# sunxiaojun2014/cilium

Hardware: AMD Instinct MI355X
Metric: Mpps classified (LPM ipcache + policy map) at 1/2/4/8 GPUs; % HBM roofline (higher is better)
Workload: dtype u32; 1 GPU; config2: 100k IPv4 ipcache LPM + 64k policy entries (4 ep x 16k), 64M-tuple batches per GPU, bit-exact verdicts; tuples_per_gpu=67108864

## Files before the change

### cilium_amd/_abi.py

```python
from __future__ import annotations

import ctypes as C
import os

HERE = os.path.dirname(os.path.abspath(__file__))
LIB_PATH = os.path.join(HERE, "libcgpu.so")

CGPU_ABI_VERSION = 2


class CgpuConfig(C.Structure):
    _fields_ = [
        ("abi_version", C.c_uint32),
        ("ipcache_max", C.c_uint32), ("policy_max_per_ep", C.c_uint32),
        ("policy_max_total", C.c_uint32), ("max_endpoints", C.c_uint32),
        ("cidr_dyn_max", C.c_uint32), ("cidr_fix_max", C.c_uint32),
        ("endpoints_max", C.c_uint32),
        ("host_id", C.c_uint32), ("world_id", C.c_uint32), ("cluster_id", C.c_uint32),
        ("health_id", C.c_uint32),
        ("ipv4_cluster_mask", C.c_uint32), ("ipv4_cluster_range", C.c_uint32),
        ("ipv6_router_ip", C.c_uint8 * 16),
        ("ct_proto_gate", C.c_uint8), ("ingress_secctx_world", C.c_uint8),
        ("prefilter_fix4", C.c_uint8), ("prefilter_dyn4", C.c_uint8),
        ("prefilter_fix6", C.c_uint8), ("prefilter_dyn6", C.c_uint8),
# ... 150 lines not shown
    "cgpu_cidr_update": (i32, [vp, i32, vp, u64]),
    "cgpu_cidr_delete": (i32, [vp, i32, vp]),
    "cgpu_cidr_lookup": (i32, [vp, i32, vp]),
    "cgpu_cidr_get_next_key": (i32, [vp, i32, vp, vp]),
    "cgpu_cidr_update_batch": (i32, [vp, i32, vp, sz, u64]),
    "cgpu_prefilter_insert": (i32, [vp, C.c_int64, vp, sz]),
    "cgpu_prefilter_delete": (i32, [vp, C.c_int64, vp, sz]),
    "cgpu_prefilter_revision": (i32, [vp, C.POINTER(C.c_int64)]),
    "cgpu_endpoint_update": (i32, [vp, vp, u64]),
    "cgpu_endpoint_delete": (i32, [vp, vp]),
    "cgpu_endpoint_lookup": (i32, [vp, vp]),
    "cgpu_endpoint_update_info": (i32, [vp, vp, vp, u64]),
    "cgpu_endpoint_lookup_info": (i32, [vp, vp, vp]),
    "cgpu_tunnel_update": (i32, [vp, vp, vp, u64]),
    "cgpu_tunnel_delete": (i32, [vp, vp]),
    "cgpu_tunnel_lookup": (i32, [vp, vp, vp]),
    "cgpu_tunnel_get_next_key": (i32, [vp, vp, vp]),
    "cgpu_tunnel_count": (sz, [vp]),
    "cgpu_forward_v4": (i32, [vp, C.POINTER(FwdParams), C.POINTER(FwdIn), sz, C.POINTER(FwdOut), vp]),
    "cgpu_forward_v6": (i32, [vp, C.POINTER(FwdParams), C.POINTER(FwdIn), sz, C.POINTER(FwdOut), vp]),
    "cgpu_forward_table_bytes": (i32, [vp, vp]),
    "cgpu_forward_frames": (i32, [vp, C.POINTER(FwdfParams), C.POINTER(FwdfIn), sz, C.POINTER(FwdOut), vp]),
    "cgpu_deliver_v4": (i32, [vp, C.POINTER(DlvIn), sz, C.POINTER(DlvOut), vp]),
    "cgpu_deliver_v6": (i32, [vp, C.POINTER(DlvIn), sz, C.POINTER(DlvOut), vp]),
    "cgpu_lb4_update": (i32, [vp, vp, vp, u64]),
    "cgpu_lb4_update_batch": (i32, [vp, vp, vp, sz, u64]),
    "cgpu_lb4_delete": (i32, [vp, vp]),
    "cgpu_lb4_lookup": (i32, [vp, vp, vp]),
    "cgpu_lb4_get_next_key": (i32, [vp, vp, vp]),
    "cgpu_lb4_count": (sz, [vp]),
    "cgpu_lb6_update": (i32, [vp, vp, vp, u64]),
    "cgpu_lb6_update_batch": (i32, [vp, vp, vp, sz, u64]),
    "cgpu_lb6_delete": (i32, [vp, vp]),
    "cgpu_lb6_lookup": (i32, [vp, vp, vp]),
    "cgpu_lb6_get_next_key": (i32, [vp, vp, vp]),
    "cgpu_lb6_count": (sz, [vp]),
    "cgpu_revnat4_update": (i32, [vp, u16, vp, u64]),
    "cgpu_revnat4_delete": (i32, [vp, u16]),
    "cgpu_revnat4_lookup": (i32, [vp, u16, vp]),
    "cgpu_revnat4_get_next_key": (i32, [vp, C.POINTER(u16), C.POINTER(u16)]),
    "cgpu_revnat4_count": (sz, [vp]),
    "cgpu_revnat6_update": (i32, [vp, u16, vp, u64]),
    "cgpu_revnat6_delete": (i32, [vp, u16]),
    "cgpu_revnat6_lookup": (i32, [vp, u16, vp]),
    "cgpu_revnat6_get_next_key": (i32, [vp, C.POINTER(u16), C.POINTER(u16)]),
    "cgpu_revnat6_count": (sz, [vp]),
    "cgpu_flow_hash6": (u32, [vp, vp, C.c_uint16, C.c_uint16, C.c_uint8]),
    "cgpu_flow_hash": (u32, [u32, u32, C.c_uint16, C.c_uint16, C.c_uint8]),
    "cgpu_commit": (i32, [vp, C.POINTER(u64)]),
    "cgpu_table_checksum": (i32, [vp, C.POINTER(u64)]),
    "cgpu_table_verify": (i32, [vp]),
    "cgpu_mirror_save": (i32, [vp, C.c_char_p]),
    "cgpu_mirror_restore": (i32, [vp, C.c_char_p]),
    "cgpu__test_corrupt": (i32, [vp, i32, sz, C.c_uint8]),
    "cgpu_counter_layout_checksum": (i32, [vp, C.POINTER(u64)]),
    "cgpu_classify_v4": (i32, [vp, C.POINTER(TuplesV4), sz, vp, vp, vp, vp]),
    "cgpu_classify_v4_host": (i32, [vp, C.POINTER(TuplesV4), sz, vp, vp, vp, vp]),
    "cgpu_classify_v6": (i32, [vp, C.POINTER(TuplesV6), sz, vp, vp, vp, vp]),
    "cgpu_classify_v4_tun": (i32, [vp, C.POINTER(TuplesV4), vp, vp, i32, sz, vp, vp, vp, vp, vp]),
    "cgpu_classify_v6_tun": (i32, [vp, C.POINTER(TuplesV6), vp, vp, i32, sz, vp, vp, vp, vp, vp]),
    "cgpu_classify_v6_lb": (i32, [vp, C.POINTER(TuplesV6), vp, vp, sz, vp, vp, vp, vp]),
    "cgpu_classify_v4_lb": (i32, [vp, C.POINTER(TuplesV4), vp, vp, sz, vp, vp, vp, vp]),
    "cgpu_classify_v4_cascade": (i32, [vp, C.POINTER(TuplesV4), vp, vp, sz, vp, vp, vp, vp]),
    "cgpu_classify_v4_lb_host": (i32, [vp, C.POINTER(TuplesV4), vp, vp, sz, vp, vp, vp, vp]),
    "cgpu_classify_v4_cascade_host": (i32, [vp, C.POINTER(TuplesV4), vp, vp, sz, vp, vp, vp, vp]),
    "cgpu_classify_v6_host": (i32, [vp, C.POINTER(TuplesV6), sz, vp, vp, vp, vp]),
    "cgpu_classify_v6_lb_host": (i32, [vp, C.POINTER(TuplesV6), vp, vp, sz, vp, vp, vp, vp]),
    "cgpu_lb4_select": (i32, [vp, i32, C.POINTER(Lb4Tuples), sz, C.POINTER(Lb4Out), vp]),
    "cgpu_prefilter_v4": (i32, [vp, vp, vp, vp, sz, vp, vp]),
    "cgpu_prefilter_v6": (i32, [vp, vp, vp, vp, sz, vp, vp]),
    "cgpu_prefilter_v4_host": (i32, [vp, vp, vp, vp, sz, vp, vp]),
    "cgpu_prefilter_v6_host": (i32, [vp, vp, vp, vp, sz, vp, vp]),
    "cgpu_lxc_update": (i32, [vp, u32, vp]),
    "cgpu_lxc_delete": (i32, [vp, u32]),
    "cgpu_lxc_lookup": (i32, [vp, u32, vp]),
    "cgpu_frames_parse": (i32, [vp, C.POINTER(Frames), sz, C.POINTER(FrameTuples), vp]),
    "cgpu_classify_frames": (i32, [vp, C.POINTER(Frames), sz, vp, vp, vp, vp]),
    "cgpu_classify_frames_host": (i32, [vp, C.POINTER(Frames), sz, vp, vp, vp, vp]),
    "cgpu_classify_frames_lb": (i32, [vp, C.POINTER(FlbIn), u32, sz, vp, vp, vp, C.POINTER(FlbOut), vp]),
    "cgpu_ct4_update": (i32, [vp, vp, vp, u64]),
    "cgpu_ct4_delete": (i32, [vp, vp]),
    "cgpu_ct4_lookup": (i32, [vp, vp, vp]),
    "cgpu_ct4_get_next_key": (i32, [vp, vp, vp]),
    "cgpu_ct4_count": (sz, [vp]),
    "cgpu_ct4_gc": (i32, [vp, u32, C.POINTER(u64)]),
    "cgpu_ct_stats": (i32, [vp, C.c_int, vp]),
    "cgpu_ct_lru_stats": (i32, [vp, C.c_int, vp]),
    "cgpu_ct4_flush": (i32, [vp]),
    "cgpu_classify_v4_ct": (i32, [vp, C.POINTER(TuplesV4Ct), sz, u32, vp, vp, vp, vp, vp]),
    "cgpu_classify_v4_ct_tun": (i32, [vp, C.POINTER(TuplesV4Ct), sz, u32, vp, vp, vp, vp, vp, vp]),
    "cgpu_classify_v6_ct_tun": (i32, [vp, C.POINTER(TuplesV6Ct), sz, u32, vp, vp, vp, vp, vp, vp]),
    "cgpu_classify_v4_ctlb": (i32, [vp, C.POINTER(TuplesV4Ct), vp, sz, u32, C.POINTER(CtlbOut), vp]),
    "cgpu_ct6_update": (i32, [vp, vp, vp, u64]),
    "cgpu_ct6_delete": (i32, [vp, vp]),
    "cgpu_ct6_lookup": (i32, [vp, vp, vp]),
    "cgpu_ct6_get_next_key": (i32, [vp, vp, vp]),
    "cgpu_ct6_count": (sz, [vp]),
    "cgpu_ct6_gc": (i32, [vp, u32, C.POINTER(u64)]),
    "cgpu_ct6_flush": (i32, [vp]),
    "cgpu_classify_v6_ctlb": (i32, [vp, C.POINTER(TuplesV6Ct), vp, sz, u32, C.POINTER(CtlbOut), vp]),
    "cgpu_classify_v6_ct": (i32, [vp, C.POINTER(TuplesV6Ct), sz, u32, vp, vp, vp, vp, vp]),
    "cgpu_classify_v4_ct_rnat": (i32, [vp, C.POINTER(TuplesV4Ct), sz, u32, vp, vp, vp, vp,
                                       C.POINTER(Rnat4Out), vp]),
    "cgpu_classify_v4_ctlb_rnat": (i32, [vp, C.POINTER(TuplesV4Ct), vp, sz, u32, C.POINTER(CtlbOut),
                                         C.POINTER(Rnat4Out), vp]),
    "cgpu_classify_v6_ct_rnat": (i32, [vp, C.POINTER(TuplesV6Ct), sz, u32, vp, vp, vp, vp,
                                       C.POINTER(Rnat6Out), vp]),
    "cgpu_classify_v6_ctlb_rnat": (i32, [vp, C.POINTER(TuplesV6Ct), vp, sz, u32, C.POINTER(CtlbOut),
                                         C.POINTER(Rnat6Out), vp]),
    "cgpu_rnat_frames_v4": (i32, [vp, C.POINTER(Rnf4In), u32, sz, vp, vp]),
    "cgpu_rnat_frames_v6": (i32, [vp, C.POINTER(Rnf6In), u32, sz, vp, vp]),
    "cgpu_frames_parse_ct": (i32, [vp, C.POINTER(Frames), sz, C.POINTER(FrameCtCols), vp]),
    "cgpu_classify_frames_ct": (i32, [vp, C.POINTER(Frames), sz, u32, C.POINTER(FctOut), vp]),
    "cgpu_l3_compile":(i32, [vp, vp, vp, vp, u32, vp]),
    "cgpu_mapstate_sync": (i32, [vp, vp, vp, vp, vp, vp]),
    "cgpu_counter_delta_bytes": (sz, [vp]),
    "cgpu_counter_bind": (i32, [vp, vp, sz]),
    "cgpu_counter_fold": (i32, [vp, vp]),
    "cgpu_metrics_read": (i32, [vp, vp]),
    "cgpu_counters_reset": (i32, [vp]),
    "cgpu_stream_release": (i32, [vp, vp]),
    "cgpu_host_stage_release": (i32, [vp]),
    "cgpu_table_bytes": (i32, [vp, vp]),
    "cgpu_host_stage_bytes": (sz, [vp]),
    "cgpu_counters_rebalance": (i32, [vp, C.POINTER(u64)]),
    "cgpu_comm_id_create": (i32, [vp]),
    "cgpu_comm_init": (i32, [vp, vp, i32, i32]),
    "cgpu_counters_allreduce": (i32, [vp, vp]),
}

_lib = None


class CgpuLibraryMissing(RuntimeError):
    pass


def lib():
    global _lib
    if _lib is None:
        if not os.path.exists(LIB_PATH):
            raise CgpuLibraryMissing(
                f"{LIB_PATH} is missing: build it with `python -m cilium_amd.build` "
                "(there is no CPU fallback for the classification path)")
        L = C.CDLL(LIB_PATH)
        for name, (res, args) in PROTOS.items():
            f = getattr(L, name)
            f.restype = res
            f.argtypes = args
        _lib = L
    return _lib


class CgpuError(OSError):
    pass


def check(rc: int, what: str) -> int:
    if rc < 0:
        msg = lib().cgpu_last_error().decode(errors="replace")
        raise CgpuError(-rc, f"{what}: {os.strerror(-rc)} ({msg})")
    return rc
```

### cilium_amd/csrc/host.cpp

```cpp
#include <hip/hip_runtime.h>
#include <rccl/rccl.h>

#include <algorithm>
#include <array>
#include <cerrno>
#include <cstdarg>
#include <cstdio>
#include <cstdlib>
#include <cstring>
#include <deque>
#include <functional>
#include <map>
#include <memory>
#include <mutex>
#include <thread>
#include <set>
#include <string>
#include <type_traits>
#include <unordered_map>
#include <vector>

#include "../../include/cgpu.h"
#include "launch.h"
#include "tables.h"
// ... 94 lines not shown
};
struct PolEntry {
	uint16_t proxy_port;
	uint32_t slot;
	uint64_t first_epoch;
};
struct SlotInit {
	uint32_t slot;
	uint64_t packets, bytes;
};

struct Dir248 {
	std::vector<uint32_t> tbl24, tbl8, vals;
	bool share = false;
	std::unordered_map<uint32_t, uint32_t> shared;
	void init() { tbl24.assign(DIR_TBL24_ENTRIES, 0u); tbl8.clear(); vals.clear(); shared.clear(); }
	uint32_t encode(uint32_t label)
	{
		if (label < (1u << DIR_TAG_SHIFT))
			return DIR_TAG_DIRECT | label;
		if (share) {
			auto it = shared.find(label);
			if (it != shared.end())
				return DIR_TAG_INDIRECT | it->second;
			shared.emplace(label, (uint32_t)vals.size());
		}
		vals.push_back(label);
		return DIR_TAG_INDIRECT | (uint32_t)(vals.size() - 1);
	}
	void apply(uint32_t addr, uint32_t len, uint32_t enc)
	{
		if (len <= 24) {
			uint32_t cnt = 1u << (24 - len);
			uint32_t base = len == 0 ? 0 : ((addr >> 8) & ~(cnt - 1));
			std::fill(tbl24.begin() + base, tbl24.begin() + base + cnt, enc);
			return;
		}
		uint32_t idx = addr >> 8, e = tbl24[idx];
		if ((e & DIR_TAG_MASK) != DIR_TAG_GROUP) {
			uint32_t g = (uint32_t)(tbl8.size() / 256);
			tbl8.resize(tbl8.size() + 256, e);
			tbl24[idx] = DIR_TAG_GROUP | g;
		}
		uint32_t g = tbl24[idx] & DIR_PAYLOAD_MASK;
		uint32_t cnt = 1u << (32 - len);
		uint32_t lo = (addr & 255u) & ~(cnt - 1);
		std::fill(tbl8.begin() + g * 256 + lo, tbl8.begin() + g * 256 + lo + cnt, enc);
	}
};

struct Lpm16cBuild {
	std::vector<uint32_t> d16, nodes, x16, dict;
	std::unordered_map<uint32_t, uint32_t> code;
	size_t nodes_at_build = 0;
	typedef std::vector<std::pair<uint32_t, uint32_t>> Runs;
	static void push(Runs &r, uint32_t start, uint32_t v)
	{
		if (r.empty() || r.back().second != v)
			r.push_back({start, v});
	}
	uint32_t emit_node(const Runs &r)
	{
		const uint32_t k = (uint32_t)r.size() - 1;
		const uint32_t kind = k <= 2 ? 0u : (k <= 4 ? 1u : 2u);
		const uint32_t nb = kind == 0 ? 1u : (kind == 1 ? 2u : 5u);
		const uint32_t words = kind == 0 ? 4u : (kind == 1 ? 8u : 16u);
		const uint32_t off = (uint32_t)(nodes.size() / 4);
		nodes.resize(nodes.size() + words, 0u);
		uint32_t *w = &nodes[(size_t)off * 4];
		for (uint32_t i = 0; i < 2 * nb; i++) {
			uint32_t b = i < k ? r[i + 1].first : 0xFFFFu;
			w[i / 2] |= (i & 1) ? (b << 16) : b;
		}
		for (uint32_t i = 0; i <= 2 * nb && nb + i < words; i++)
			w[nb + i] = r[std::min<uint32_t>(i, k)].second;
		return DIR_TAG_GROUP | (kind << LPMC_KIND_SHIFT) | off;
	}
	uint32_t emit_array(const uint32_t *ent)
	{
		const uint32_t off = (uint32_t)(nodes.size() / 4);
		nodes.insert(nodes.end(), ent, ent + 256);
		return DIR_TAG_GROUP | (3u << LPMC_KIND_SHIFT) | off;
	}
	uint32_t byte_level(const uint32_t *leaf)
	{
		Runs r;
		for (uint32_t j = 0; j < 256; j++)
			push(r, j, leaf[j]);
		if (r.size() == 1)
			return r[0].second;
		if (r.size() - 1 <= LPMC_MAX_RUN_BOUNDS)
			return emit_node(r);
		return emit_array(leaf);
	}
	static Runs runs16(uint32_t p, const std::vector<uint32_t> &tbl24, const std::vector<uint32_t> &tbl8)
	{
		Runs r;
		const uint32_t *t = &tbl24[(size_t)p * 256];
		for (uint32_t j = 0; j < 256 && r.size() <= LPMC_MAX_RUN_BOUNDS + 1; j++) {
			if ((t[j] & DIR_TAG_MASK) != DIR_TAG_GROUP) {
				push(r, j << 8, t[j]);
				continue;
			}
			const uint32_t *g = &tbl8[(size_t)(t[j] & DIR_PAYLOAD_MASK) * 256];
			for (uint32_t b = 0; b < 256; b++)
				push(r, (j << 8) | b, g[b]);
		}
		return r;
	}
	uint32_t entry16(uint32_t p, const Runs &r, const std::vector<uint32_t> &tbl24,
			 const std::vector<uint32_t> &tbl8)
	{
		if (r.size() == 1)
			return r[0].second;
		if (r.size() - 1 <= LPMC_MAX_RUN_BOUNDS)
			return emit_node(r);
		const uint32_t *t = &tbl24[(size_t)p * 256];
		uint32_t ent[256];
		for (uint32_t j = 0; j < 256; j++)
			ent[j] = (t[j] & DIR_TAG_MASK) != DIR_TAG_GROUP
					 ? t[j]
					 : byte_level(&tbl8[(size_t)(t[j] & DIR_PAYLOAD_MASK) * 256]);
		return emit_array(ent);
	}
	void inline16(uint32_t p, const Runs &r)
	{
		uint32_t *w = &x16[(size_t)p * 4];
		w[0] = w[1] = w[2] = w[3] = 0;
		bool inl = r.size() <= 5;
		for (size_t i = 0; inl && i < r.size(); i++)
			inl = code.count(r[i].second) != 0;
		if (!inl) {
			w[0] = d16[p];
			w[3] = LPMC_OVERFLOW;
			return;
		}
		const uint32_t k = (uint32_t)r.size() - 1;
		uint64_t v = 0;
		for (uint32_t i = 0; i < 4; i++) {
			uint32_t b = i < k ? r[i + 1].first : 0xFFFFu;
			w[i / 2] |= (i & 1) ? (b << 16) : b;
		}
		for (uint32_t i = 0; i < 5; i++)
			v |= (uint64_t)code.at(r[std::min(i, k)].second) << (12 * i);
		w[2] = (uint32_t)v;
		w[3] = (uint32_t)(v >> 32);
	}
	void build(const std::vector<uint32_t> &tbl24, const std::vector<uint32_t> &tbl8)
	{
		d16.assign(65536, 0u);
		nodes.clear();
		std::vector<Runs> all(65536);
		for (uint32_t p = 0; p < 65536; p++) {
			all[p] = runs16(p, tbl24, tbl8);
			d16[p] = entry16(p, all[p], tbl24, tbl8);
		}
		std::map<uint32_t, uint64_t> freq;
		for (auto &r : all)
			if (r.size() <= 5)
				for (auto &x : r)
					freq[x.second]++;
		std::vector<std::pair<uint64_t, uint32_t>> byf;
		for (auto &kv : freq)
			byf.push_back({kv.second, kv.first});
		std::sort(byf.begin(), byf.end(), [](const std::pair<uint64_t, uint32_t> &a,
						     const std::pair<uint64_t, uint32_t> &b) {
			return a.first != b.first ? a.first > b.first : a.second < b.second;
		});
		dict.clear();
		code.clear();
		for (auto &f : byf) {
			if (dict.size() >= LPMC_DICT)
				break;
			code[f.second] = (uint32_t)dict.size();
			dict.push_back(f.second);
		}
		x16.assign((size_t)65536 * 4, 0u);
		for (uint32_t p = 0; p < 65536; p++)
			inline16(p, all[p]);
		nodes_at_build = nodes.size();
	}
	void patch(uint32_t lo, uint32_t hi, const std::vector<uint32_t> &tbl24, const std::vector<uint32_t> &tbl8)
	{
		for (uint32_t p = lo; p <= hi; p++) {
			const Runs r = runs16(p, tbl24, tbl8);
			d16[p] = entry16(p, r, tbl24, tbl8);
			if (r.size() <= 5)
				for (auto &x : r)
					if (!code.count(x.second) && dict.size() < LPMC_DICT) {
						code[x.second] = (uint32_t)dict.size();
						dict.push_back(x.second);
					}
			inline16(p, r);
		}
	}
	bool bloated() const { return nodes.size() > 2 * nodes_at_build + (1u << 16); }
};

struct Rank4 {
	uint32_t rank;
	uint32_t addr;
	uint32_t len;
	uint32_t label;
	uint32_t tunnel;
};

struct Arena {
	std::vector<std::pair<const void *, size_t>> parts;
	std::vector<size_t> offs;
	size_t total = 0;
	size_t add(const void *src, size_t bytes)
	{
		size_t off = (total + 255) & ~(size_t)255;
		parts.push_back({src, bytes});
		offs.push_back(off);
		total = off + bytes;
		return off;
	}
};

}

namespace {

uint64_t fnv(uint64_t h, const void *p, size_t n)
{
	const uint8_t *b = (const uint8_t *)p;
	for (size_t i = 0; i < n; i++)
		h = (h ^ b[i]) * 0x100000001b3ull;
	return h;
}

static const uint8_t kStaticV4[4] = {0, 0, 0, 1};
bool ipc4_candidate(const cgpu_ipcache_key &raw, uint32_t label, Rank4 *r)
{
	const uint32_t p = raw.prefixlen;
	const uint8_t *data = (const uint8_t *)&raw + 4;
	if (p > 64 || !prefix_eq(data, kStaticV4, std::min<uint32_t>(p, 32)))
		return false;
	r->label = label;
	r->rank = p;
	if (p < 32) {
		r->addr = 0;
		r->len = 0;
	} else {
		r->len = p - 32;
		uint32_t a;
		memcpy(&a, data + 4, 4);
		r->addr = bswap32(a) & (r->len ? ~0u << (32 - r->len) : 0u);
// ... 3920 lines not shown
	if (!c)
		return fail(-EINVAL, "null argument");
	if (c->device < 0)
		return fail(-ENODEV, "context has no device");
	std::lock_guard<std::mutex> cg(c->commit_mu);
	std::shared_ptr<Epoch> e;
	{
		std::lock_guard<std::mutex> g(c->pub_mu);
		e = c->cur;
	}
	if (!e)
		return fail(-ENOENT, "nothing committed");
	HIP_OR_EIO(hipSetDevice(c->device));
	HIP_OR_EIO(hipMemsetAsync(c->d_verify, 0, (G_N + 1) * 8, c->ustream));
	for (int k = 0; k < G_N; k++)
		if (e->bufs[k])
			for (auto &pt : e->bufs[k]->parts)
				HIP_OR_EIO(launch_table_sum(e->bufs[k]->p, pt.first, pt.second, c->d_verify + k,
							    c->ustream));
	uint64_t got[G_N + 1];
	HIP_OR_EIO(hipMemcpyAsync(got, c->d_verify, sizeof(got), hipMemcpyDeviceToHost, c->ustream));
	HIP_OR_EIO(hipStreamSynchronize(c->ustream));
	static const char *names[G_N] = {"ipcache", "policy", "prefilter", "endpoints", "lb4", "lxc", "lb6"};
	for (int k = 0; k < G_N; k++)
		if (e->bufs[k] && got[k] != e->bufs[k]->host_sum)
			return fail(-EIO, "device %s tables differ from the host image (sum %016llx, expected %016llx)",
				    names[k], (unsigned long long)got[k], (unsigned long long)e->bufs[k]->host_sum);
	return 0;
}

CGPU_EXPORT int cgpu__test_corrupt(cgpu_ctx *c, int group, size_t off, uint8_t mask)
{
	if (!c || c->device < 0 || group < 0 || group >= G_N)
		return -EINVAL;
	std::shared_ptr<Epoch> e;
	{
		std::lock_guard<std::mutex> g(c->pub_mu);
		e = c->cur;
	}
	if (!e || !e->bufs[group] || off >= e->bufs[group]->bytes)
		return -EINVAL;
	uint8_t b;
	HIP_OR_EIO(hipSetDevice(c->device));
	HIP_OR_EIO(hipDeviceSynchronize());
	HIP_OR_EIO(hipMemcpy(&b, (char *)e->bufs[group]->p + off, 1, hipMemcpyDeviceToHost));
	b ^= mask;
	HIP_OR_EIO(hipMemcpy((char *)e->bufs[group]->p + off, &b, 1, hipMemcpyHostToDevice));
	return 0;
}

static uint32_t lpmc_host_lookup(const Lpm16cBuild &t, uint32_t h)
{
	const uint32_t *q = &t.x16[(size_t)(h >> 16) * 4];
	if (!(q[3] & LPMC_OVERFLOW)) {
		const uint32_t x = h & 0xFFFFu;
		const uint32_t cnt = (x >= (q[0] & 0xFFFFu)) + (x >= (q[0] >> 16)) + (x >= (q[1] & 0xFFFFu)) +
				     (x >= (q[1] >> 16));
		const uint64_t v = ((uint64_t)q[3] << 32) | q[2];
		return t.dict[(uint32_t)(v >> (12u * cnt)) & 0xFFFu];
	}
	const uint32_t ARR = (DIR_TAG_GROUP >> LPMC_KIND_SHIFT) | 3u;
	uint32_t e = q[0];
	bool lvl8 = false;
	if ((e >> LPMC_KIND_SHIFT) == ARR) {
		e = t.nodes[(size_t)(e & LPMC_OFF_MASK) * 4u + ((h >> 8) & 255u)];
		lvl8 = true;
		if ((e >> LPMC_KIND_SHIFT) == ARR)
			e = t.nodes[(size_t)(e & LPMC_OFF_MASK) * 4u + (h & 255u)];
	}
	if ((e & DIR_TAG_MASK) == DIR_TAG_GROUP) {
		const uint32_t kind = (e >> LPMC_KIND_SHIFT) & 3u;
		const uint32_t nb = kind == 0 ? 1u : (kind == 1 ? 2u : 5u);
		const uint32_t *w = &t.nodes[(size_t)(e & LPMC_OFF_MASK) * 4u];
		const uint32_t x = lvl8 ? (h & 255u) : (h & 0xFFFFu);
		uint32_t cnt = 0;
		for (uint32_t i = 0; i < nb; i++)
			cnt += (x >= (w[i] & 0xFFFFu)) + (x >= (w[i] >> 16));
		e = w[nb + cnt];
	}
	return e;
}

static uint32_t leaf_value(const std::vector<uint32_t> &vals, uint32_t e)
{
	return (e & DIR_TAG_MASK) == DIR_TAG_INDIRECT ? vals[e & DIR_PAYLOAD_MASK] : e & DIR_PAYLOAD_MASK;
}

static int diag_ipc_compile(const cgpu_ipcache_key *keys, const cgpu_remote_endpoint_info *vals,
			    const uint8_t *del, size_t n, size_t n_first, cgpu_ctx **out)
{
	cgpu_config cfg;
	cgpu_config_default(&cfg);
	cfg.ipcache_tunnel = 1;
	cfg.ipcache_max = (uint32_t)std::max<size_t>(n, 1);
	cgpu_ctx *c = nullptr;
	*out = nullptr;
	if (int r = cgpu_ctx_create(&cfg, -1, &c))
		return r;
	*out = c;
	int rc = 0;
	for (int phase = 0; phase < 2 && !rc; phase++) {
		const size_t lo = phase ? n_first : 0, hi = phase ? n : n_first;
		if (phase && lo == hi)
			break;
		for (size_t i = lo; i < hi && !rc; i++) {
			rc = del && del[i] ? cgpu_ipcache_delete(c, &keys[i]) : cgpu_ipcache_update(c, &keys[i], &vals[i], CGPU_ANY);
// ... 55 lines not shown
		return fail(-EINVAL, "null argument");
	std::lock_guard<std::mutex> cg(c->commit_mu);
	out[0] = c->b.ipc_builds;
	out[1] = c->b.ipc_patched;
	return 0;
}

static void lpmc_shapes(const Lpm16cBuild &t, uint32_t *o)
{
	const uint32_t GRP = DIR_TAG_GROUP >> LPMC_KIND_SHIFT;
	o[0] = (uint32_t)t.dict.size();
	o[15] = (uint32_t)t.nodes.size();
	if (t.x16.empty())
		return;
	for (uint32_t p = 0; p < 65536; p++) {
		const uint32_t *q = &t.x16[(size_t)p * 4];
		if (!(q[3] & LPMC_OVERFLOW)) {
			const uint64_t v = ((uint64_t)q[3] << 32) | q[2];
			uint32_t starts = 0;
			for (uint32_t i = 0; i < 4; i++)
				starts += ((v >> (12u * i)) & 0xFFFu) != ((v >> (12u * (i + 1))) & 0xFFFu);
			o[1 + starts]++;
			continue;
		}
		const uint32_t e = q[0];
		if ((e & DIR_TAG_MASK) != DIR_TAG_GROUP) {
			o[6]++;
			continue;
		}
		const uint32_t kind = (e >> LPMC_KIND_SHIFT) & 3u;
		o[7 + kind]++;
		if (kind != 3u)
			continue;
		const uint32_t *a = &t.nodes[(size_t)(e & LPMC_OFF_MASK) * 4u];
		for (uint32_t j = 0; j < 256; j++)
			if ((a[j] >> LPMC_KIND_SHIFT & ~3u) == GRP)
				o[11 + ((a[j] >> LPMC_KIND_SHIFT) & 3u)]++;
	}
}

CGPU_EXPORT int cgpu_diag_ipc4_shapes(const cgpu_ipcache_key *keys, const cgpu_remote_endpoint_info *vals,
				      const uint8_t *del, size_t n, size_t n_first, uint32_t *out, uint64_t *commits)
{
	if ((n && (!keys || !vals)) || !out || n_first > n)
		return fail(-EINVAL, "null argument");
	cgpu_ctx *c = nullptr;
	const int rc = diag_ipc_compile(keys, vals, del, n, n_first, &c);
	if (!c)
		return rc;
	memset(out, 0, 32 * sizeof(uint32_t));
	if (!rc) {
		lpmc_shapes(c->b.lc, out);
		lpmc_shapes(c->b.lcT, out + 16);
	}
	if (commits) {
		commits[0] = c->b.ipc_builds;
		commits[1] = c->b.ipc_patched;
	}
	cgpu_ctx_destroy(c);
	return rc;
}

CGPU_EXPORT int cgpu_diag_pol_tables(const uint32_t *eps, const cgpu_policy_key *keys,
				     const cgpu_policy_entry *entries, const uint8_t *del, size_t n,
				     size_t n_first, uint32_t *rows, uint64_t *stats)
{
	if ((n && (!eps || !keys || !entries || !rows)) || !stats || n_first > n)
		return fail(-EINVAL, "null argument");
	cgpu_config cfg;
	cgpu_config_default(&cfg);
	cgpu_ctx *c = nullptr;
	if (int r = cgpu_ctx_create(&cfg, -1, &c))
		return r;
	int rc = 0;
	uint64_t reloc[2] = {0, 0};
	for (int phase = 0; phase < 2 && !rc; phase++) {
		const size_t lo = phase ? n_first : 0, hi = phase ? n : n_first;
		if (phase && lo == hi)
			break;
		for (size_t i = lo; i < hi && !rc; i++)
			rc = del && del[i] ? cgpu_policy_delete(c, eps[i], &keys[i])
					   : cgpu_policy_update(c, eps[i], &keys[i], &entries[i], CGPU_ANY);
		if (rc)
			break;
		CommitIn in;
		in.cfg = c->cfg;
		{
			std::lock_guard<std::mutex> g(c->mu);
			capture_pol(c, in, c->b);
		}
		const uint64_t before = c->b.pol.relocations;
		compile_pol(c, in);
		reloc[phase] = c->b.pol.relocations - before;
	}
	BuildState &b = c->b;
	for (size_t i = 0; i < n && !rc; i++) {
		uint32_t *r = rows + 4 * i;
		r[0] = r[1] = r[2] = r[3] = ~0u;
		const uint64_t k64 = pol_key64(&keys[i]);
		PolEntry pe;
		{
			std::lock_guard<std::mutex> g(c->mu);
			auto it = c->pol[eps[i]].find(k64);
			if (it == c->pol[eps[i]].end())
				continue;
			pe = it->second;
// ... 3281 lines not shown
```

### cilium_amd/csrc/kernels.hip

```cpp
#include "cgpu.h"
#include "launch.h"

#include <algorithm>
#include <cstdlib>
#include <cstring>
#include <map>
#include <mutex>
#include <tuple>

#define DROP_POLICY (-133)
#define DROP_CT_UNKNOWN_PROTO (-137)
#define DROP_NO_SERVICE (-158)
#define XDP_DROP 1
#define XDP_PASS 2
#define VERDICT_XDP_DROP (-4097)
#define TC_ACT_OK 0
#define TC_ACT_REDIRECT 7

namespace {

constexpr int BLOCK = 256;

__device__ __forceinline__ uint32_t bswap32(uint32_t x) { return __builtin_bswap32(x); }

// ... 2013 lines not shown
#pragma unroll
			for (int u = 0; u < Q; u++) {
				te[u] = 0u;
				twant[u] = (fw[u] & (F_OK | F_GATED | F_LBDROP | F_EG)) == (F_OK | F_EG);
			}
		}
		if (V6) {
			bool act[Q];
#pragma unroll
			for (int u = 0; u < Q; u++)
				act[u] = (fw[u] & (F_OK | F_GATED | F_LBDROP)) == F_OK;
#ifdef CGPU_DIAG_V6_NO_TRIE
#pragma unroll
			for (int u = 0; u < Q; u++)
				e[u] = act[u] ? (DIR_TAG_DIRECT | 2u) : 0u;
#else
			if constexpr (IPCE) {
				uint32_t pe[QA];
				if (full && Q == 4) {
					const uint4 v = ld_x4<NTL>(a.ipc_e + i0);
					pe[0] = v.x, pe[1] = v.y, pe[2] = v.z, pe[3] = v.w;
				} else if (full && Q == 2) {
					const uint2 v = ld_x2<NTL>(a.ipc_e + i0);
					pe[0] = v.x, pe[1] = v.y;
				} else {
#pragma unroll
					for (int u = 0; u < Q; u++)
						pe[u] = a.ipc_e[i0 + u < a.n ? i0 + u : i0];
				}
#pragma unroll
				for (int u = 0; u < Q; u++)
					e[u] = act[u] ? pe[u] : 0u;
			} else {
				if constexpr (TUN) {
#pragma unroll
					for (int u = 0; u < Q; u++)
						if (twant[u])
							te[u] = v6_lookup(ta.t.t6, v6_host_words(ad6[u]));
				}
				v6t_lookup_q<Q>(s.ipc6, ldict, n24 != 0u, ad6, act, e);
			}
#endif
		} else {
			if constexpr (QX) {
				uint4 q[Q];
				bool act[Q];
#pragma unroll
				for (int u = 0; u < Q; u++) {
					act[u] = (fw[u] & (F_OK | F_GATED | F_LBDROP)) == F_OK;
					q[u] = reinterpret_cast<const uint4 *>(
						s.ipc4c.x16)[act[u] ? DIAG_LPM(bswap32(ad[u]) >> 16) : 0u];
				}
				whole_q<Q>(q);
#pragma unroll
				for (int u = 0; u < Q; u++) {
					const bool inl = act[u] && !(q[u].w & LPMC_OVERFLOW);
					const uint32_t x = bswap32(ad[u]) & 0xFFFFu;
					const uint32_t cnt = (x >= (q[u].x & 0xFFFFu) ? 1u : 0u) + (x >= (q[u].x >> 16) ? 1u : 0u) +
							     (x >= (q[u].y & 0xFFFFu) ? 1u : 0u) + (x >= (q[u].y >> 16) ? 1u : 0u);
					const uint64_t v = ((uint64_t)q[u].w << 32) | q[u].z;
					const uint32_t leaf = ldict[inl ? (uint32_t)(v >> (12u * cnt)) & 0xFFFu : 0u];
					e[u] = !act[u] ? 0u : (inl ? leaf : q[u].x);
				}
			} else {
				uint4 q[Q];
				uint4 tq[TUN ? Q : 1];
#pragma unroll
				for (int u = 0; u < Q; u++) {
					q[u] = make_uint4(0, 0, 0, 0);
					if ((fw[u] & (F_OK | F_GATED | F_LBDROP)) == F_OK)
						q[u] = reinterpret_cast<const uint4 *>(s.ipc4c.x16)[DIAG_LPM(bswap32(ad[u]) >> 16)];
					if constexpr (TUN) {
						tq[u] = make_uint4(0, 0, 0, 0);
						if (twant[u])
							tq[u] = reinterpret_cast<const uint4 *>(ta.t.t4.x16)[bswap32(ad[u]) >> 16];
					}
				}
				if constexpr (TUN) {
#pragma unroll
					for (int u = 0; u < Q; u++) {
						if (!twant[u] || (tq[u].w & LPMC_OVERFLOW))
							continue;
						const uint32_t x = bswap32(ad[u]) & 0xFFFFu;
						const uint32_t cnt = (x >= (tq[u].x & 0xFFFFu) ? 1u : 0u) + (x >= (tq[u].x >> 16) ? 1u : 0u) +
								     (x >= (tq[u].y & 0xFFFFu) ? 1u : 0u) + (x >= (tq[u].y >> 16) ? 1u : 0u);
						const uint64_t v = ((uint64_t)tq[u].w << 32) | tq[u].z;
						te[u] = ta.t.t4.dict[(uint32_t)(v >> (12u * cnt)) & 0xFFFu];
					}
#pragma unroll
					for (int u = 0; u < Q; u++)
						if (twant[u] && (tq[u].w & LPMC_OVERFLOW))
							te[u] = lpmc_lookup(ta.t.t4, ta.t.t4.dict, ad[u]);
				}
#pragma unroll
				for (int u = 0; u < Q; u++) {
					if (q[u].w & LPMC_OVERFLOW) {
						e[u] = q[u].x;
						continue;
					}
					const uint32_t x = bswap32(ad[u]) & 0xFFFFu;
					const uint32_t cnt = (x >= (q[u].x & 0xFFFFu) ? 1u : 0u) + (x >= (q[u].x >> 16) ? 1u : 0u) +
							     (x >= (q[u].y & 0xFFFFu) ? 1u : 0u) + (x >= (q[u].y >> 16) ? 1u : 0u);
					const uint64_t v = ((uint64_t)q[u].w << 32) | q[u].z;
					e[u] = (fw[u] & (F_OK | F_GATED | F_LBDROP)) == F_OK ? ldict[(uint32_t)(v >> (12u * cnt)) & 0xFFFu] : 0u;
				}
			}
			{
				constexpr uint32_t ARR = (DIR_TAG_GROUP >> LPMC_KIND_SHIFT) | 3u;
#pragma unroll
				for (int u = 0; u < Q; u++)
					if ((e[u] >> LPMC_KIND_SHIFT) == ARR) {
						e[u] = s.ipc4c.nodes[(size_t)(e[u] & LPMC_OFF_MASK) * 4u +
								     ((bswap32(ad[u]) >> 8) & 255u)];
						fw[u] |= F_LVL8;
					}
#pragma unroll
				for (int u = 0; u < Q; u++)
					if ((e[u] >> LPMC_KIND_SHIFT) == ARR)
						e[u] = s.ipc4c.nodes[(size_t)(e[u] & LPMC_OFF_MASK) * 4u + (bswap32(ad[u]) & 255u)];
				if constexpr (QX) {
					bool grpn[Q], far[Q], anyn = false, anyf = false;
					uint32_t kind[Q], idx[Q];
#pragma unroll
					for (int u = 0; u < Q; u++) {
						grpn[u] = (e[u] & DIR_TAG_MASK) == DIR_TAG_GROUP;
						kind[u] = grpn[u] ? (e[u] >> LPMC_KIND_SHIFT) & 3u : 0u;
						anyn |= grpn[u];
					}
					if (__ballot(anyn)) {
						uint4 q[Q][2];
#pragma unroll
						for (int u = 0; u < Q; u++) {
							const uint4 *nd = grpn[u] ? reinterpret_cast<const uint4 *>(s.ipc4c.nodes) +
											    (e[u] & LPMC_OFF_MASK)
										  : reinterpret_cast<const uint4 *>(s.ipc4c.x16);
							q[u][0] = nd[0];
							q[u][1] = nd[kind[u] ? 1 : 0];
						}
#pragma unroll
						for (int u = 0; u < Q; u++) {
							const uint32_t w[8] = {q[u][0].x, q[u][0].y, q[u][0].z, q[u][0].w,
									       q[u][1].x, q[u][1].y, q[u][1].z, q[u][1].w};
							const uint32_t h = bswap32(ad[u]);
							const uint32_t x = (fw[u] & F_LVL8) ? (h & 255u) : (h & 0xFFFFu);
							const uint32_t nb = kind[u] == 0 ? 1u : (kind[u] == 1 ? 2u : 5u);
							uint32_t cnt = 0;
#pragma unroll
							for (uint32_t i = 0; i < 5; i++)
								if (i < nb)
									cnt += (x >= (w[i] & 0xFFFFu) ? 1u : 0u) + (x >= (w[i] >> 16) ? 1u : 0u);
							idx[u] = nb + cnt;
							uint32_t r = w[1];
#pragma unroll
							for (uint32_t j = 2; j < 8; j++)
								r = j == idx[u] ? w[j] : r;
							far[u] = grpn[u] && idx[u] >= 8u;
							anyf |= far[u];
							if (grpn[u] && !far[u])
								e[u] = r;
						}
						if (__ballot(anyf)) {
							uint32_t r[Q];
#pragma unroll
							for (int u = 0; u < Q; u++)
								r[u] = *(far[u] ? s.ipc4c.nodes + (size_t)(e[u] & LPMC_OFF_MASK) * 4u + idx[u]
										: s.ipc4c.x16);
#pragma unroll
							for (int u = 0; u < Q; u++)
								e[u] = far[u] ? r[u] : e[u];
						}
					}
				} else {
				uint4 q[Q][2];
#pragma unroll
				for (int u = 0; u < Q; u++) {
					q[u][0] = q[u][1] = make_uint4(0, 0, 0, 0);
					if ((e[u] & DIR_TAG_MASK) == DIR_TAG_GROUP) {
						const uint4 *nd = reinterpret_cast<const uint4 *>(s.ipc4c.nodes) +
								  (e[u] & LPMC_OFF_MASK);
						q[u][0] = nd[0];
						if ((e[u] >> LPMC_KIND_SHIFT) & 3u)
							q[u][1] = nd[1];
					}
				}
#pragma unroll
				for (int u = 0; u < Q; u++) {
					if ((e[u] & DIR_TAG_MASK) != DIR_TAG_GROUP)
						continue;
					const uint32_t kind = (e[u] >> LPMC_KIND_SHIFT) & 3u;
					uint4 q2 = make_uint4(0, 0, 0, 0), q3 = q2;
// ... 6742 lines not shown
```

### cilium_amd/csrc/tables.h

```cpp
#ifndef CGPU_TABLES_H
#define CGPU_TABLES_H

#include <stdint.h>

#define DIR_TAG_SHIFT 30u
#define DIR_TAG_MASK (3u << DIR_TAG_SHIFT)
#define DIR_TAG_DIRECT (1u << DIR_TAG_SHIFT)
#define DIR_TAG_GROUP (2u << DIR_TAG_SHIFT)
#define DIR_TAG_INDIRECT (3u << DIR_TAG_SHIFT)
#define DIR_PAYLOAD_MASK ((1u << DIR_TAG_SHIFT) - 1u)
#define DIR_TBL24_ENTRIES (1u << 24)

#define LPMC_KIND_SHIFT 28u
#define LPMC_OFF_MASK ((1u << LPMC_KIND_SHIFT) - 1u)
#define LPMC_MAX_RUN_BOUNDS 10u

#define LPMC_DICT 4095u
#define LPMC_OVERFLOW (1u << 31)

typedef struct lpm16c {
	const uint32_t *d16;
	const uint32_t *nodes;
	const uint32_t *vals;
	const uint32_t *x16;
	const uint32_t *dict;
	uint32_t n_node_words;
	uint32_t n_dict;
} lpm16c;

static inline __host__ __device__ uint32_t mix32(uint32_t a, uint32_t b)
{
	uint64_t h = ((uint64_t)b << 32 | a) * 0x9E3779B97F4A7C15ull;
	h ^= h >> 29;
	h *= 0xbf58476d1ce4e5b9ull;
	h ^= h >> 32;
	return (uint32_t)h;
}

#define POL_HOP 8u
#define POL_HOP_SHIFT 24u
#define POL_CTR_MASK 0x00FFFFFFu
#define POL_CTR_EMPTY POL_CTR_MASK

typedef struct pol_slot {
	uint32_t key_lo;
	uint32_t key_hi;
	uint32_t ep_proxy;
	uint32_t ctr;
} pol_slot;

typedef struct pol_table {
	const pol_slot *slots;
	uint32_t bucket_mask;
	uint32_t pad_;
} pol_table;

#define PG_EGRESS (1u << 16)
#define PG_USED (1u << 17)

typedef struct pol_groups {
	const uint4 *slots;
	uint32_t mask;
	uint32_t pad_;
} pol_groups;

static inline __host__ __device__ uint32_t pg_hash(uint32_t id, uint32_t ep_dir)
{
	return mix32(id, ep_dir ^ 0x6a09e667u);
}

static inline __host__ __device__ uint32_t pg_bloom(uint32_t dport, uint32_t proto)
// ... 314 lines not shown
```

Before: 46940 Mpps.

## Split overflowing /16 LPM buckets into inline child nodes resolved by a second gather

```diff
diff --git a/cilium_amd/_abi.py b/cilium_amd/_abi.py
--- a/cilium_amd/_abi.py
+++ b/cilium_amd/_abi.py
@@ -226,8 +226,7 @@
     "cgpu_table_verify": (i32, [vp]),
     "cgpu_mirror_save": (i32, [vp, C.c_char_p]),
     "cgpu_mirror_restore": (i32, [vp, C.c_char_p]),
-    "cgpu__test_corrupt": (i32, [vp, i32, sz, C.c_uint8]),
-    "cgpu_counter_layout_checksum": (i32, [vp, C.POINTER(u64)]),
+    "cgpu__test_corrupt": (i32, [vp, i32, sz, C.c_uint8]),    "cgpu_counter_layout_checksum": (i32, [vp, C.POINTER(u64)]),
     "cgpu_classify_v4": (i32, [vp, C.POINTER(TuplesV4), sz, vp, vp, vp, vp]),
     "cgpu_classify_v4_host": (i32, [vp, C.POINTER(TuplesV4), sz, vp, vp, vp, vp]),
     "cgpu_classify_v6": (i32, [vp, C.POINTER(TuplesV6), sz, vp, vp, vp, vp]),
@@ -303,6 +302,10 @@
     "cgpu_counters_allreduce": (i32, [vp, vp]),
 }
 
+TEST_HOOKS = {
+    "cgpu_diag_ipc4_split": (i32, [vp, vp, vp, sz, sz, vp, vp]),
+}
+
 _lib = None
 
 
@@ -322,6 +325,10 @@
             f = getattr(L, name)
             f.restype = res
             f.argtypes = args
+        for name, (res, args) in TEST_HOOKS.items():
+            f = getattr(L, name, None)
+            if f is not None:
+                f.restype, f.argtypes = res, args
         _lib = L
     return _lib
 
diff --git a/cilium_amd/csrc/host.cpp b/cilium_amd/csrc/host.cpp
--- a/cilium_amd/csrc/host.cpp
+++ b/cilium_amd/csrc/host.cpp
@@ -170,7 +170,7 @@
 struct Lpm16cBuild {
 	std::vector<uint32_t> d16, nodes, x16, dict;
 	std::unordered_map<uint32_t, uint32_t> code;
-	size_t nodes_at_build = 0;
+	size_t nodes_at_build = 0, kids_at_build = 0;
 	typedef std::vector<std::pair<uint32_t, uint32_t>> Runs;
 	static void push(Runs &r, uint32_t start, uint32_t v)
 	{
@@ -215,7 +215,7 @@
 	{
 		Runs r;
 		const uint32_t *t = &tbl24[(size_t)p * 256];
-		for (uint32_t j = 0; j < 256 && r.size() <= LPMC_MAX_RUN_BOUNDS + 1; j++) {
+		for (uint32_t j = 0; j < 256 && r.size() <= LPMC_SPLIT_MAX_RUNS; j++) {
 			if ((t[j] & DIR_TAG_MASK) != DIR_TAG_GROUP) {
 				push(r, j << 8, t[j]);
 				continue;
@@ -241,6 +241,44 @@
 					 : byte_level(&tbl8[(size_t)(t[j] & DIR_PAYLOAD_MASK) * 256]);
 		return emit_array(ent);
 	}
+	size_t kid_words() const { return x16.size() > (size_t)65536 * 4 ? x16.size() - (size_t)65536 * 4 : 0; }
+	void inline_node(uint32_t *w, const Runs &r, size_t at, uint32_t n)
+	{
+		const uint32_t k = n - 1;
+		uint64_t v = 0;
+		w[0] = w[1] = 0;
+		for (uint32_t i = 0; i < 4; i++) {
+			uint32_t b = i < k ? r[at + i + 1].first : 0xFFFFu;
+			w[i / 2] |= (i & 1) ? (b << 16) : b;
+		}
+		for (uint32_t i = 0; i < 5; i++)
+			v |= (uint64_t)code.at(r[at + std::min(i, k)].second) << (12 * i);
+		w[2] = (uint32_t)v;
+		w[3] = (uint32_t)(v >> 32);
+	}
+	void split16(uint32_t p, const Runs &r)
+	{
+		const size_t n = r.size();
+		if (n < 6 || n > LPMC_SPLIT_MAX_RUNS)
+			return;
+		for (auto &x : r)
+			if (!code.count(x.second))
+				return;
+		const uint32_t nch = (uint32_t)(n + 4) / 5;
+		const size_t base = x16.size() / 4;
+		if (base + nch - 1 > LPMC_SPLIT_BASE_MASK)
+			return;
+		x16.resize(x16.size() + (size_t)nch * 4, 0u);
+		uint32_t *w = &x16[(size_t)p * 4];
+		w[1] = w[2] = 0xFFFFFFFFu;
+		for (uint32_t j = 1; j < nch; j++) {
+			const uint32_t c = r[(size_t)5 * j].first, sh = (j - 1) & 1 ? 16u : 0u;
+			w[1 + (j - 1) / 2] = (w[1 + (j - 1) / 2] & ~(0xFFFFu << sh)) | (c << sh);
+		}
+		for (uint32_t j = 0; j < nch; j++)
+			inline_node(&x16[(base + j) * 4], r, (size_t)5 * j, (uint32_t)std::min<size_t>(5, n - (size_t)5 * j));
+		w[3] = LPMC_OVERFLOW | LPMC_SPLIT | ((nch - 1) << LPMC_SPLIT_LAST_SHIFT) | (uint32_t)base;
+	}
 	void inline16(uint32_t p, const Runs &r)
 	{
 		uint32_t *w = &x16[(size_t)p * 4];
@@ -251,18 +289,10 @@
 		if (!inl) {
 			w[0] = d16[p];
 			w[3] = LPMC_OVERFLOW;
+			split16(p, r);
 			return;
 		}
-		const uint32_t k = (uint32_t)r.size() - 1;
-		uint64_t v = 0;
-		for (uint32_t i = 0; i < 4; i++) {
-			uint32_t b = i < k ? r[i + 1].first : 0xFFFFu;
-			w[i / 2] |= (i & 1) ? (b << 16) : b;
-		}
-		for (uint32_t i = 0; i < 5; i++)
-			v |= (uint64_t)code.at(r[std::min(i, k)].second) << (12 * i);
-		w[2] = (uint32_t)v;
-		w[3] = (uint32_t)(v >> 32);
+		inline_node(w, r, 0, (uint32_t)r.size());
 	}
 	void build(const std::vector<uint32_t> &tbl24, const std::vector<uint32_t> &tbl8)
 	{
@@ -297,6 +327,7 @@
 		for (uint32_t p = 0; p < 65536; p++)
 			inline16(p, all[p]);
 		nodes_at_build = nodes.size();
+		kids_at_build = kid_words();
 	}
 	void patch(uint32_t lo, uint32_t hi, const std::vector<uint32_t> &tbl24, const std::vector<uint32_t> &tbl8)
 	{
@@ -312,7 +343,10 @@
 			inline16(p, r);
 		}
 	}
-	bool bloated() const { return nodes.size() > 2 * nodes_at_build + (1u << 16); }
+	bool bloated() const
+	{
+		return nodes.size() + kid_words() > 2 * (nodes_at_build + kids_at_build) + (1u << 16);
+	}
 };
 
 struct Rank4 {
@@ -4339,6 +4373,13 @@
 static uint32_t lpmc_host_lookup(const Lpm16cBuild &t, uint32_t h)
 {
 	const uint32_t *q = &t.x16[(size_t)(h >> 16) * 4];
+	if ((q[3] & (LPMC_OVERFLOW | LPMC_SPLIT)) == (LPMC_OVERFLOW | LPMC_SPLIT)) {
+		const uint32_t x = h & 0xFFFFu;
+		const uint32_t k = (x >= (q[1] & 0xFFFFu)) + (x >= (q[1] >> 16)) + (x >= (q[2] & 0xFFFFu)) +
+				   (x >= (q[2] >> 16));
+		q = &t.x16[((size_t)(q[3] & LPMC_SPLIT_BASE_MASK) +
+			    std::min(k, (q[3] >> LPMC_SPLIT_LAST_SHIFT) & 7u)) * 4];
+	}
 	if (!(q[3] & LPMC_OVERFLOW)) {
 		const uint32_t x = h & 0xFFFFu;
 		const uint32_t cnt = (x >= (q[0] & 0xFFFFu)) + (x >= (q[0] >> 16)) + (x >= (q[1] & 0xFFFFu)) +
@@ -4500,6 +4541,51 @@
 	if (!rc) {
 		lpmc_shapes(c->b.lc, out);
 		lpmc_shapes(c->b.lcT, out + 16);
+	}
+	if (commits) {
+		commits[0] = c->b.ipc_builds;
+		commits[1] = c->b.ipc_patched;
+	}
+	cgpu_ctx_destroy(c);
+	return rc;
+}
+
+static void lpmc_split_counts(const Lpm16cBuild &t, const Dir248 &d, uint32_t *o)
+{
+	if (t.x16.empty())
+		return;
+	o[6] = (uint32_t)t.kid_words();
+	for (uint32_t p = 0; p < 65536; p++) {
+		const uint32_t *q = &t.x16[(size_t)p * 4];
+		if (!(q[3] & LPMC_OVERFLOW))
+			continue;
+		if (q[3] & LPMC_SPLIT) {
+			const uint32_t last = (q[3] >> LPMC_SPLIT_LAST_SHIFT) & 7u;
+			o[last - 1]++;
+			o[7] += (last + 1) * 4;
+			continue;
+		}
+		const size_t starts = Lpm16cBuild::runs16(p, d.tbl24, d.tbl8).size() - 1;
+		if (starts >= LPMC_SPLIT_MAX_RUNS)
+			o[5]++;
+		else if (starts >= 5)
+			o[4]++;
+	}
+}
+
+CGPU_EXPORT int cgpu_diag_ipc4_split(const cgpu_ipcache_key *keys, const cgpu_remote_endpoint_info *vals,
+				     const uint8_t *del, size_t n, size_t n_first, uint32_t *out, uint64_t *commits)
+{
+	if ((n && (!keys || !vals)) || !out || n_first > n)
+		return fail(-EINVAL, "null argument");
+	cgpu_ctx *c = nullptr;
+	const int rc = diag_ipc_compile(keys, vals, del, n, n_first, &c);
+	if (!c)
+		return rc;
+	memset(out, 0, 16 * sizeof(uint32_t));
+	if (!rc) {
+		lpmc_split_counts(c->b.lc, c->b.dir, out);
+		lpmc_split_counts(c->b.lcT, c->b.dirT, out + 8);
 	}
 	if (commits) {
 		commits[0] = c->b.ipc_builds;
diff --git a/cilium_amd/csrc/kernels.hip b/cilium_amd/csrc/kernels.hip
--- a/cilium_amd/csrc/kernels.hip
+++ b/cilium_amd/csrc/kernels.hip
@@ -2089,15 +2089,36 @@
 						s.ipc4c.x16)[act[u] ? DIAG_LPM(bswap32(ad[u]) >> 16) : 0u];
 				}
 				whole_q<Q>(q);
+				uint4 c[Q];
+				bool spl[Q], inl[Q];
+				uint32_t w0[Q], ci[Q];
 #pragma unroll
 				for (int u = 0; u < Q; u++) {
-					const bool inl = act[u] && !(q[u].w & LPMC_OVERFLOW);
+					inl[u] = act[u] && !(q[u].w & LPMC_OVERFLOW);
+					spl[u] = act[u] && (q[u].w & (LPMC_OVERFLOW | LPMC_SPLIT)) == (LPMC_OVERFLOW | LPMC_SPLIT);
 					const uint32_t x = bswap32(ad[u]) & 0xFFFFu;
 					const uint32_t cnt = (x >= (q[u].x & 0xFFFFu) ? 1u : 0u) + (x >= (q[u].x >> 16) ? 1u : 0u) +
 							     (x >= (q[u].y & 0xFFFFu) ? 1u : 0u) + (x >= (q[u].y >> 16) ? 1u : 0u);
+					const uint32_t k = (x >= (q[u].y & 0xFFFFu) ? 1u : 0u) + (x >= (q[u].y >> 16) ? 1u : 0u) +
+							   (x >= (q[u].z & 0xFFFFu) ? 1u : 0u) + (x >= (q[u].z >> 16) ? 1u : 0u);
+					const uint32_t last = (q[u].w >> LPMC_SPLIT_LAST_SHIFT) & 7u;
 					const uint64_t v = ((uint64_t)q[u].w << 32) | q[u].z;
-					const uint32_t leaf = ldict[inl ? (uint32_t)(v >> (12u * cnt)) & 0xFFFu : 0u];
-					e[u] = !act[u] ? 0u : (inl ? leaf : q[u].x);
+					ci[u] = spl[u] ? (q[u].w & LPMC_SPLIT_BASE_MASK) + (k < last ? k : last) : 0u;
+					w0[u] = inl[u] ? (uint32_t)(v >> (12u * cnt)) & 0xFFFu : q[u].x;
+				}
+#pragma unroll
+				for (int u = 0; u < Q; u++)
+					c[u] = reinterpret_cast<const uint4 *>(s.ipc4c.x16)[ci[u]];
+				whole_q<Q>(c);
+#pragma unroll
+				for (int u = 0; u < Q; u++) {
+					const uint32_t x = bswap32(ad[u]) & 0xFFFFu;
+					const uint32_t cnt = (x >= (c[u].x & 0xFFFFu) ? 1u : 0u) + (x >= (c[u].x >> 16) ? 1u : 0u) +
+							     (x >= (c[u].y & 0xFFFFu) ? 1u : 0u) + (x >= (c[u].y >> 16) ? 1u : 0u);
+					const uint64_t v = ((uint64_t)c[u].w << 32) | c[u].z;
+					const uint32_t code = spl[u] ? (uint32_t)(v >> (12u * cnt)) & 0xFFFu : w0[u];
+					const uint32_t leaf = ldict[inl[u] || spl[u] ? code : 0u];
+					e[u] = !act[u] ? 0u : (inl[u] || spl[u] ? leaf : w0[u]);
 				}
 			} else {
 				uint4 q[Q];
@@ -2142,8 +2163,44 @@
 					e[u] = (fw[u] & (F_OK | F_GATED | F_LBDROP)) == F_OK ? ldict[(uint32_t)(v >> (12u * cnt)) & 0xFFFu] : 0u;
 				}
 			}
+#ifdef CGPU_DIAG_LPM_ONE_GATHER
+			if constexpr (QX) {
+				bool grpn[Q], anyn = false;
+#pragma unroll
+				for (int u = 0; u < Q; u++) {
+					grpn[u] = (e[u] & DIR_TAG_MASK) == DIR_TAG_GROUP;
+					anyn |= grpn[u];
+				}
+				if (__ballot(anyn)) {
+					uint4 q[Q];
+#pragma unroll
+					for (int u = 0; u < Q; u++) {
+						const uint32_t kind = (e[u] >> LPMC_KIND_SHIFT) & 3u;
+						q[u] = *(grpn[u] ? reinterpret_cast<const uint4 *>(s.ipc4c.nodes) +
+									   (e[u] & LPMC_OFF_MASK) + (kind == 1u || kind == 2u ? 1 : 0)
+								 : reinterpret_cast<const uint4 *>(s.ipc4c.x16));
+					}
+					whole_q<Q>(q);
+#pragma unroll
+					for (int u = 0; u < Q; u++) {
+						const uint32_t r = (q[u].y & DIR_TAG_MASK) == DIR_TAG_GROUP
+									   ? DIR_TAG_DIRECT | (q[u].y & 0xFFFFu)
+									   : q[u].y;
+						e[u] = grpn[u] ? r : e[u];
+					}
+				}
+			} else
+#endif
 			{
 				constexpr uint32_t ARR = (DIR_TAG_GROUP >> LPMC_KIND_SHIFT) | 3u;
+				bool anya = !QX;
+				if constexpr (QX) {
+#pragma unroll
+					for (int u = 0; u < Q; u++)
+						anya |= (e[u] >> LPMC_KIND_SHIFT) == ARR;
+					anya = __ballot(anya) != 0;
+				}
+				if (anya) {
 #pragma unroll
 				for (int u = 0; u < Q; u++)
 					if ((e[u] >> LPMC_KIND_SHIFT) == ARR) {
@@ -2155,6 +2212,7 @@
 				for (int u = 0; u < Q; u++)
 					if ((e[u] >> LPMC_KIND_SHIFT) == ARR)
 						e[u] = s.ipc4c.nodes[(size_t)(e[u] & LPMC_OFF_MASK) * 4u + (bswap32(ad[u]) & 255u)];
+				}
 				if constexpr (QX) {
 					bool grpn[Q], far[Q], anyn = false, anyf = false;
 					uint32_t kind[Q], idx[Q];
@@ -2172,7 +2230,7 @@
 											    (e[u] & LPMC_OFF_MASK)
 										  : reinterpret_cast<const uint4 *>(s.ipc4c.x16);
 							q[u][0] = nd[0];
-							q[u][1] = nd[kind[u] ? 1 : 0];
+							q[u][1] = *(kind[u] ? nd + 1 : reinterpret_cast<const uint4 *>(s.ipc4c.x16));
 						}
 #pragma unroll
 						for (int u = 0; u < Q; u++) {
diff --git a/cilium_amd/csrc/tables.h b/cilium_amd/csrc/tables.h
--- a/cilium_amd/csrc/tables.h
+++ b/cilium_amd/csrc/tables.h
@@ -17,6 +17,10 @@
 
 #define LPMC_DICT 4095u
 #define LPMC_OVERFLOW (1u << 31)
+#define LPMC_SPLIT (1u << 30)
+#define LPMC_SPLIT_LAST_SHIFT 27u
+#define LPMC_SPLIT_BASE_MASK ((1u << LPMC_SPLIT_LAST_SHIFT) - 1u)
+#define LPMC_SPLIT_MAX_RUNS 25u
 
 typedef struct lpm16c {
 	const uint32_t *d16;
```

Measured after the change: 55910 Mpps (median of 6 runs). 1.19x the previous value.
